# schmidtniko/visual_marker_mapping

Measured on AMD Instinct MI355X. Metric: lm_iterations_per_sec, higher is better.
Workload: dtype f64; 1 GPU; configs[1]: 500 images x 200 tags, visibility 1.00, 100000 tag observations (400000 corner residual blocks), no loss, perturbed initial guess; eliminated_family=cameras, reduced_system_order=1200, elimination_form=dense Z + MFMA rank-k, kept_family_order=natural

## Files before the change

visual_marker_mapping_amd/csrc/kernels_chol.hip:

```cpp
#include <type_traits>
#include <utility>

#include "engine.hpp"

namespace vmm {

#ifdef VMM_STAMPS
__device__ unsigned long long g_stamps[64];
#define STAMP(slot)                                                                  \
    do {                                                                             \
        if (blockIdx.x == 1 && threadIdx.x == 0 && k == 1) {                         \
            g_stamps[slot] = __builtin_amdgcn_s_memtime();                           \
            g_stamps[16 + slot] = __builtin_amdgcn_s_memrealtime();                  \
        }                                                                            \
    } while (0)
#define USTAMP(slot)                                                                 \
    do {                                                                             \
        if (u == 0 && threadIdx.x == 0 && k == 1 && t == u + n_wg)                   \
            g_stamps[(slot)] = __builtin_amdgcn_s_memtime();                         \
    } while (0)
#else
#define USTAMP(slot)
#define STAMP(slot)
#endif
// ... 731 lines not shown
            L[r * kLd + cc] = (cc <= r) ? Ld[(int64_t)kb * 4096 + r * 64 + cc] : 0.0;
        }
        if (tid < 64)
            di[tid] = dinv[K0 + tid];
    }
    __syncthreads();
    if (part == 0) {
        wc = w[m * kNB + c];
        if (kb + 1 < n_blk) {
            wc -= (red[0][c] + red[1][c]) + (red[2][c] + red[3][c]);
            w[m * kNB + c] = wc;
        }
    }
    if (m != kb)
        return;
    double yj = 0.0;
    for (int j0 = 60; j0 >= 0; j0 -= 4) {
        if (part == 0)
            ws[c] = wc;
        __syncthreads();
        if (part == 0) {
            const double* D = L + j0 * kLd + j0;
            const double v3 = ws[j0 + 3] * di[j0 + 3];
            const double v2 = (ws[j0 + 2] - D[3 * kLd + 2] * v3) * di[j0 + 2];
            const double v1 = (ws[j0 + 1] - D[2 * kLd + 1] * v2 - D[3 * kLd + 1] * v3) * di[j0 + 1];
            const double v0 = (ws[j0] - D[kLd] * v1 - D[2 * kLd] * v2 - D[3 * kLd] * v3) * di[j0];
            if (c >= j0 && c < j0 + 4)
                yj = (c == j0) ? v0 : (c == j0 + 1 ? v1 : (c == j0 + 2 ? v2 : v3));
            if (c < j0)
                wc -= L[j0 * kLd + c] * v0 + L[(j0 + 1) * kLd + c] * v1 + L[(j0 + 2) * kLd + c] * v2
                    + L[(j0 + 3) * kLd + c] * v3;
        }
        __syncthreads();
    }
    if (part == 0)
        y[kb * kNB + c] = yj;
}

constexpr unsigned kSpinLimit = 1u << 22;

__device__ __forceinline__ void raise_sync_timeout(LmCtl* ctl, int bit)
{
    atomicOr(&ctl->sync_timeout, bit);
    atomicExch(&ctl->done, 2);
}

int backsolve_chain_workgroups(int n_blk) { return n_blk; }

__device__ __forceinline__ void chain_block_done(unsigned* n_done, int n_blk, unsigned* epoch_word, unsigned epoch,
                                                 bool tree, int m)
{
    if (!tree) {
        if (m == 0)
            *epoch_word = epoch;
        return;
    }
    if (atomicAdd(n_done, 1u) == (unsigned)n_blk - 1u) {
        *n_done = 0u;
        *epoch_word = epoch;
    }
}

#ifdef VMM_STAMPS
__device__ unsigned long long g_chain_stamps[128][4];
#define CH_RT(blk, slot)                                                                  \
    do {                                                                                  \
        if (threadIdx.x == 0)                                                             \
            g_chain_stamps[(blk) & 127][slot] = __builtin_amdgcn_s_memrealtime();         \
    } while (0)
extern "C" int vmm_ba_debug_read_chain_stamps(unsigned long long* out)
{
    return (int)hipMemcpyFromSymbol(out, HIP_SYMBOL(g_chain_stamps), sizeof(unsigned long long) * 128 * 4);
}
#else
#define CH_RT(blk, slot)
#endif

__global__ __launch_bounds__(256) void k_backsolve_chain(LmCtl* ctl, const double* __restrict__ S, int ld,
                                                         int n_pad, int n_blk, double* y,
                                                         const double* __restrict__ dinv, unsigned long long* gran,
                                                         unsigned* epoch_word, const double* __restrict__ Ld,
                                                         const double* __restrict__ Linv)
{
    if (ctl->done || ctl->lin_fail) {
        if (blockIdx.x == gridDim.x - 1 && threadIdx.x == 0)
            *epoch_word = *epoch_word + 1u;
        return;
    }
    const unsigned spin_limit = (ctl->spin_limit_chain && (ctl->spin_wg < 0 || ctl->spin_wg == (int)blockIdx.x))
                                    ? ctl->spin_limit_chain : kSpinLimit;
    __shared__ double L[64 * kLd];
    __shared__ double Li[64 * kLd];
    __shared__ double red[4][64];
    __shared__ double ws[64];
    __shared__ double ys[2][64];
    __shared__ double sB[16][256];
    __shared__ int s_timeout;
    const int m = n_blk - 1 - (int)blockIdx.x;
    const int tid = threadIdx.x;
    const int c = tid & 63, part = tid >> 6;
    const unsigned epoch = *epoch_word + 1u;
    const int K0 = m * kNB;
    if (tid == 0)
        s_timeout = 0;
    CH_RT(m, 0);
    auto receive = [&](const int j, double* ysj) {
        if (part == 0) {
            const unsigned long long* g = gran + 2 * (int64_t)(j * kNB + c);
            unsigned long long x0, x1;
            for (unsigned n = 0;;) {
                x0 = __hip_atomic_load(g, __ATOMIC_RELAXED, __HIP_MEMORY_SCOPE_AGENT);
                x1 = __hip_atomic_load(g + 1, __ATOMIC_RELAXED, __HIP_MEMORY_SCOPE_AGENT);
                const bool ok = (unsigned)(x0 >> 32) == epoch && (unsigned)(x1 >> 32) == epoch;
                if (__all(ok) && spin_limit != 1u)
                    break;
                __builtin_amdgcn_s_sleep(1);
                if (++n >= spin_limit) {
                    s_timeout = 1;
                    break;
                }
            }
            ysj[c] = __longlong_as_double((long long)(((x1 & 0xffffffffull) << 32) | (x0 & 0xffffffffull)));
        }
    };
    auto publish = [&](const double yv) {
        const unsigned long long bits = (unsigned long long)__double_as_longlong(yv);
        const unsigned long long tag = (unsigned long long)epoch << 32;
        unsigned long long* g = gran + 2 * (int64_t)(K0 + c);
        __hip_atomic_store(g, tag | (bits & 0xffffffffull), __ATOMIC_RELAXED, __HIP_MEMORY_SCOPE_AGENT);
        __hip_atomic_store(g + 1, tag | (bits >> 32), __ATOMIC_RELAXED, __HIP_MEMORY_SCOPE_AGENT);
        y[K0 + c] = yv;
    };
    if (m == n_blk - 1) {
        if (part == 0) {
            double lcol[64];
#pragma unroll
            for (int jj = 0; jj < 64; ++jj)
                lcol[jj] = (c <= jj) ? Ld[(int64_t)m * 4096 + jj * 64 + c] : 0.0;
            const double dic = dinv[K0 + c];
            double wv = S[(int64_t)n_pad * ld + K0 + c];
            double yv = 0.0;
#pragma unroll
            for (int jj = 63; jj >= 0; --jj) {
                const long long wb = __double_as_longlong(wv * dic);
                const unsigned w0 = (unsigned)__builtin_amdgcn_readlane((int)wb, jj);
                const unsigned w1 = (unsigned)__builtin_amdgcn_readlane((int)(wb >> 32), jj);
                const double yj = __longlong_as_double((long long)(((unsigned long long)w1 << 32) | w0));
                yv = (c == jj) ? yj : yv;
                wv = (c < jj) ? wv - lcol[jj] * yj : wv;
            }
            publish(yv);
        }
        CH_RT(m, 2);
        if (tid == 0 && m == 0)
            *epoch_word = epoch;
        return;
    }
    double li[16];
    {
        for (int idx = tid; idx < 64 * 64; idx += 256) {
            const int r = idx >> 6, cc = idx & 63;
            L[r * kLd + cc] = S[(int64_t)((m + 1) * kNB + r) * ld + K0 + cc];
            Li[r * kLd + cc] = Linv[(int64_t)m * 4096 + r * 64 + cc];
        }
        __syncthreads();
#pragma unroll
        for (int r = 0; r < 16; ++r)
            li[r] = Li[(part * 16 + r) * kLd + c];
        const int fi = c & 15, fk = c >> 4;
        double4_t accB[4];
#pragma unroll
        for (int t = 0; t < 4; ++t)
            accB[t] = (double4_t){ 0.0, 0.0, 0.0, 0.0 };
#pragma unroll
        for (int ks = 0; ks < 16; ++ks) {
            const double av = L[(part * 16 + fi) * kLd + 4 * ks + fk];
#pragma unroll
            for (int t = 0; t < 4; ++t)
                accB[t] = __builtin_amdgcn_mfma_f64_16x16x4f64(av, Li[(4 * ks + fk) * kLd + 16 * t + fi], accB[t], 0, 0, 0);
        }
#pragma unroll
        for (int t = 0; t < 4; ++t)
#pragma unroll
            for (int r = 0; r < 4; ++r)
                sB[fk + 4 * r][part * 64 + 16 * t + fi] = accB[t][r];
        __syncthreads();
    }
    double acc = 0.0;
    double lt[16], ln[16];
    int j = n_blk - 1;
    if (j > m + 1) {
        const double* Lb = S + (int64_t)(j * kNB + part * 16) * ld + K0 + c;
#pragma unroll
        for (int r = 0; r < 16; ++r)
            lt[r] = Lb[(int64_t)r * ld];
    }
    for (; j > m + 1; --j) {
        if (j - 1 > m + 1) {
            const double* Lb = S + (int64_t)((j - 1) * kNB + part * 16) * ld + K0 + c;
#pragma unroll
            for (int r = 0; r < 16; ++r)
                ln[r] = Lb[(int64_t)r * ld];
        }
        double* ysj = ys[j & 1];
        receive(j, ysj);
        __syncthreads();
#pragma unroll
        for (int r = 0; r < 16; ++r)
            acc += lt[r] * ysj[part * 16 + r];
#pragma unroll
        for (int r = 0; r < 16; ++r)
            lt[r] = ln[r];
    }
    red[part][c] = acc;
    __syncthreads();
    if (part == 0)
        ws[c] = S[(int64_t)n_pad * ld + K0 + c] - ((red[0][c] + red[1][c]) + (red[2][c] + red[3][c]));
    __syncthreads();
    double a2 = 0.0;
#pragma unroll
    for (int r = 0; r < 16; ++r)
        a2 += li[r] * ws[part * 16 + r];
    __syncthreads();
// ... 1515 lines not shown
```

visual_marker_mapping_amd/csrc/kernels_lm.hip:

```cpp
#include <float.h>

#include "engine.hpp"

namespace vmm {

__device__ __forceinline__ void control_reduce(double (&v)[8], double (&m)[2], double* sh)
{
    const int lane = threadIdx.x & 63, wave = threadIdx.x >> 6;
    const int nw = blockDim.x >> 6;
#pragma unroll
    for (int level = 0; level < 3; ++level) {
        const int off = 32 >> level;
        const bool hi = (lane & off) != 0;
#pragma unroll
        for (int j = 0; j < (4 >> level); ++j) {
            const double keep = hi ? v[2 * j + 1] : v[2 * j];
            const double send = hi ? v[2 * j] : v[2 * j + 1];
            v[j] = keep + __shfl_xor(send, off, 64);
        }
    }
#pragma unroll
    for (int off = 4; off >= 1; off >>= 1)
        v[0] += __shfl_xor(v[0], off, 64);
    {
// ... 270 lines not shown
            else
                c.num_unsuccessful++;
            if (c.records < c.trace_capacity)
                trace[c.records] = cur;
            c.records++;
            if (cur.iteration >= c.max_num_iterations) {
                stop = 1;
                c.termination = VMM_BA_NO_CONVERGENCE;
            } else if (cur.step_is_successful && cur.gradient_max_norm <= c.gradient_tolerance) {
                stop = 1;
                c.termination = VMM_BA_CONVERGENCE;
            } else if (c.radius <= c.min_radius) {
                stop = 1;
                c.termination = VMM_BA_CONVERGENCE;
            }
            if (stop) {
                c.done = 1;
            } else {
                vmm_ba_iteration z;
                z.iteration = cur.iteration + 1;
                z.step_is_valid = 0;
                z.step_is_successful = 0;
                z.reserved = 0;
                z.cost = c.x_cost;
                z.cost_change = 0.0;
                z.gradient_max_norm = cur.gradient_max_norm;
                z.step_norm = 0.0;
                z.relative_decrease = 0.0;
                z.trust_region_radius = 0.0;
                z.model_cost_change = 0.0;
                c.cur = z;
                c.iteration = z.iteration;
                c.lin_fail = 0;
                c.num_lm_iterations++;
            }
        }
        s_stop = stop;
        s_accept = accept;
        s_moved = moved;
        s_reuse = c.reuse_diagonal;
        s_radius = c.radius;
        s_lo = c.min_lm_diagonal;
        s_hi = c.max_lm_diagonal;
        if (!stop)
            c.reuse_diagonal = 1;
        else
            c.phase_ticks[1] += span(t_begin, __builtin_amdgcn_s_memrealtime());
        CTL_RT(3);
        *ctl = c;
        CTL_RT(4);
    }
    __syncthreads();
    CTL_RT(5);
    if (s_accept) {
        for (int i = tid; i < 7 * pv.n_cams; i += (int)blockDim.x)
            pv.cam_qt[i] = pv.cam_cand[i];
        for (int i = tid; i < 7 * pv.n_tags; i += (int)blockDim.x)
            pv.tag_qt[i] = pv.tag_cand[i];
    }
    if (staged && s_moved)
        for (size_t i = tid; i < small_count; i += blockDim.x)
            dst[i] = src[i];
    if (s_stop)
        return;
    const double* __restrict__ Hx = s_moved ? Hn : H0 + (which ? alt_off : 0);
    const double lo = s_lo, hi = s_hi;
    for (int q = tid; q < n_tan; q += (int)blockDim.x) {
        double d;
        if (!s_reuse) {
            const int p = q / 6, k = q % 6;
            const double sc = scale[q];
            d = sc * sc * Hx[36 * (int64_t)p + 7 * k];
            d = fmin(fmax(d, lo), hi);
            diag[q] = d;
        } else {
            d = diag[q];
        }
        const double lm = sqrt(d / s_radius);
        D2[q] = lm * lm;
    }
    CTL_RT(6);
}

__device__ __forceinline__ void candidate_for_pose(const PoseViews& pv, const int p, const double (&d)[6],
                                                   double* __restrict__ delta, const double* __restrict__ H,
                                                   const double* __restrict__ g, const int32_t* __restrict__ active,
                                                   double* __restrict__ pose_part)
{
    double bad = 0.0;
#pragma unroll
    for (int k = 0; k < 6; ++k) {
        delta[6 * (int64_t)p + k] = d[k];
        if (!isfinite(d[k]))
            bad = 1.0;
    }
    const double* x = pose_ptr(pv, p, false);
    double out[7];
    block_plus(pv, p, x, d, out);
    double* c = pose_ptr(pv, p, true);
    double sn = 0.0, xn = 0.0;
    for (int k = 0; k < 7; ++k) {
        c[k] = out[k];
        const double df = x[k] - out[k];
        sn += df * df;
        xn += out[k] * out[k];
    }
    const double* Hp = H + 36 * (int64_t)p;
    double gd = 0.0, quad = 0.0;
    for (int a = 0; a < 6; ++a) {
        gd += d[a] * g[6 * (int64_t)p + a];
        double r = 0.0;
        for (int b = 0; b < 6; ++b)
            r += Hp[6 * a + b] * d[b];
        quad += d[a] * r;
    }
    const bool act = active[p] != 0;
    double* o = pose_part + 5 * (int64_t)p;
    o[0] = gd;
    o[1] = quad;
    o[2] = act ? sn : 0.0;
    o[3] = act ? xn : 0.0;
    o[4] = bad;
}

template <bool FUSE, bool SPARSE>
__global__ __launch_bounds__(256) void k_backsub(const LmCtl* ctl, int n_e, int e_off_pose,
                                                 const int32_t* __restrict__ pose_task,
                                                 const double* __restrict__ Z, int ldz, int n_red,
                                                 const double* __restrict__ yf, const double* __restrict__ Le,
                                                 const double* __restrict__ ze, const double* __restrict__ scale,
                                                 double* __restrict__ step_comm, double* __restrict__ part_cross,
                                                 PoseViews pv, int f_off_pose, int n_f, int nb_e,
                                                 double* __restrict__ delta, const double* __restrict__ H0,
                                                 const double* __restrict__ g0, const int64_t alt_off,
                                                 const int32_t* __restrict__ active,
                                                 double* __restrict__ pose_part,
                                                 const int32_t* __restrict__ e_start,
                                                 const int32_t* __restrict__ e_other,
                                                 const int32_t* __restrict__ row_of)
{
    if (!FUSE && blockIdx.x == 0 && threadIdx.x == 0)
        step_comm[7 * (int64_t)n_e] = (ctl->done == 2) ? 1.0 : 0.0;
    if (ctl->done)
        return;
    phase_stamp(ctl, 4);
    const bool lin_fail = ctl->lin_fail != 0;
    const double* __restrict__ H = H0 + small_sel(ctl, alt_off);
    const double* __restrict__ g = g0 + small_sel(ctl, alt_off);
    if (FUSE && (int)blockIdx.x >= nb_e) {
        const int f = ((int)blockIdx.x - nb_e) * blockDim.x + threadIdx.x;
        if (f >= n_f)
            return;
        const int p = f_off_pose + f;
        double d[6];
#pragma unroll
        for (int k = 0; k < 6; ++k)
            d[k] = lin_fail ? 0.0 : -yf[(row_of ? row_of[f] : 6 * f) + k] * scale[6 * (int64_t)p + k];
        candidate_for_pose(pv, p, d, delta, H, g, active, pose_part);
        return;
    }
    const int e = (int)blockIdx.x;
    const int lane = threadIdx.x & 63, wave = threadIdx.x >> 6;
    if (e >= n_e)
        return;
    const bool owned = pose_task[e + 1] > pose_task[e];
    if (!owned || lin_fail) {
        if (wave != 0)
            return;
        if (lane < 6)
            step_comm[6 * (int64_t)e + lane] = 0.0;
        if (lane == 0) {
            part_cross[e] = 0.0;
            if (FUSE) {
                const double d[6] = { 0.0, 0.0, 0.0, 0.0, 0.0, 0.0 };
                candidate_for_pose(pv, e_off_pose + e, d, delta, H, g, active, pose_part);
            }
        }
        return;
    }
    __shared__ double s_acc[4][6];
    double acc[6] = { 0, 0, 0, 0, 0, 0 };
    if (SPARSE) {
        const int es = e_start[e], rs = 6 * (e_start[e + 1] - es);
        const double* zp = Z + 36 * (int64_t)es;
        for (int t = (int)threadIdx.x; t < rs; t += 256) {
            const int k = t / 6, c = t - 6 * k;
            const int fo = e_other[es + k];
            const double yv = yf[(row_of ? row_of[fo] : 6 * fo) + c];
#pragma unroll
            for (int i = 0; i < 6; ++i)
                acc[i] += zp[36 * k + 6 * c + i] * yv;
        }
    } else {
        const double* zr = Z + (int64_t)(6 * e) * ldz;
        for (int c = 2 * (int)threadIdx.x; c < n_red; c += 512) {
            const double2 yv = *reinterpret_cast<const double2*>(yf + c);
#pragma unroll
            for (int i = 0; i < 6; ++i) {
                const double2 zv = *reinterpret_cast<const double2*>(zr + (int64_t)i * ldz + c);
                acc[i] += zv.x * yv.x + zv.y * yv.y;
            }
        }
    }
#pragma unroll
    for (int i = 0; i < 6; ++i) {
        const double a = wave_sum(acc[i]);
        if (lane == 0)
            s_acc[wave][i] = a;
    }
    __syncthreads();
    if (wave != 0)
        return;
    double v[6];
    double cr = 0.0;
#pragma unroll
    for (int i = 0; i < 6; ++i) {
        const double a = (s_acc[0][i] + s_acc[1][i]) + (s_acc[2][i] + s_acc[3][i]);
        v[i] = ze[6 * (int64_t)e + i] - a;
        cr += v[i] * a;
    }
    const double* L = Le + 36 * (int64_t)e;
#pragma unroll
    for (int i = 5; i >= 0; --i) {
        double s = v[i];
#pragma unroll
        for (int k = i + 1; k < 6; ++k)
            s -= L[6 * k + i] * v[k];
        v[i] = s / L[6 * i + i];
    }
    double d[6];
#pragma unroll
    for (int i = 0; i < 6; ++i)
        d[i] = -v[i] * scale[6 * (int64_t)(e_off_pose + e) + i];
    if (lane < 6) {
        double out = 0.0;
#pragma unroll
        for (int i = 0; i < 6; ++i)
            out = (lane == i) ? d[i] : out;
        step_comm[6 * (int64_t)e + lane] = out;
    }
    if (lane == 0) {
        part_cross[e] = cr;
        if (FUSE)
            candidate_for_pose(pv, e_off_pose + e, d, delta, H, g, active, pose_part);
    }
}

__global__ void k_candidate(LmCtl* ctl, PoseViews pv, int n_e, int e_off_pose, int f_off_pose,
                            const double* __restrict__ step_comm, const double* __restrict__ yf,
                            const double* __restrict__ scale, double* __restrict__ delta,
                            const double* __restrict__ H, const double* __restrict__ g,
                            const int32_t* __restrict__ active, double* __restrict__ pose_part,
                            const int32_t* __restrict__ row_of)
{
    const bool remote = step_comm[7 * (int64_t)n_e] > 0.0;
    if (remote && blockIdx.x == 0 && threadIdx.x == 0 && ctl->done != 1) {
        if (ctl->done == 0)
            atomicOr(&ctl->sync_timeout, 4);
        atomicExch(&ctl->done, 2);
    }
    if (ctl->done || remote)
        return;
    const int p = blockIdx.x * blockDim.x + threadIdx.x;
    const int n_pose = pv.n_cams + pv.n_tags;
    if (p >= n_pose)
        return;
    const bool is_e = (p >= e_off_pose) && (p < e_off_pose + n_e);
    double d[6];
    for (int k = 0; k < 6; ++k) {
        if (ctl->lin_fail)
            d[k] = 0.0;
        else if (is_e)
            d[k] = step_comm[6 * (int64_t)(p - e_off_pose) + k];
        else
            d[k] = -yf[(row_of ? row_of[p - f_off_pose] : 6 * (p - f_off_pose)) + k] * scale[6 * (int64_t)p + k];
    }
    candidate_for_pose(pv, p, d, delta, H, g, active, pose_part);
}

__global__ __launch_bounds__(256) void k_begin_loop(LmCtl* ctl, const LmCtl init, const int n_cam7, const int n_tag7,
                                                    const double* __restrict__ stage_cam,
                                                    const double* __restrict__ stage_tag, double* __restrict__ cam_qt,
                                                    double* __restrict__ tag_qt, double* __restrict__ cam_cand,
                                                    double* __restrict__ tag_cand)
{
    const int i = blockIdx.x * blockDim.x + threadIdx.x;
    if (i == 0)
        *ctl = init;
    if (i < n_cam7) {
        double v;
        if (stage_cam) {
            v = stage_cam[i];
            cam_qt[i] = v;
        } else {
            v = cam_qt[i];
        }
        cam_cand[i] = v;
    } else if (i < n_cam7 + n_tag7) {
        const int k = i - n_cam7;
        double v;
        if (stage_tag) {
            v = stage_tag[k];
            tag_qt[k] = v;
        } else {
            v = tag_qt[k];
        }
        tag_cand[k] = v;
    }
}

void launch_begin_loop(Engine& e, const LmCtl& init)
{
    const int n_cam7 = 7 * e.n_cams, n_tag7 = 7 * e.n_tags;
    const double* sc = e.dirty_cam ? e.pose_stage_dev : nullptr;
    const double* st = e.dirty_tag ? e.pose_stage_dev + n_cam7 : nullptr;
    hipLaunchKernelGGL(k_begin_loop, dim3((n_cam7 + n_tag7 + 255) / 256), dim3(256), 0, e.stream, e.ctl, init, n_cam7,
                       n_tag7, sc, st, e.cam_qt, e.tag_qt, e.cam_cand, e.tag_cand);
}

__global__ void k_pose_plus(int64_t n, const double* __restrict__ qt, const double* __restrict__ delta,
                            double* __restrict__ out)
{
    const int64_t i = (int64_t)blockIdx.x * blockDim.x + threadIdx.x;
    if (i >= n)
        return;
    double x[7], d[6], o[7];
    for (int k = 0; k < 7; ++k)
// ... 98 lines not shown
```

visual_marker_mapping_amd/csrc/kernels_schur.hip:

```cpp
#include "engine.hpp"

namespace vmm {


__device__ __forceinline__ bool chol6(double* A)
{
    bool ok = true;
#pragma unroll
    for (int j = 0; j < 6; ++j) {
        double d = A[6 * j + j];
#pragma unroll
        for (int k = 0; k < j; ++k)
            d -= A[6 * j + k] * A[6 * j + k];
        if (!(d > 0.0) || !isfinite(d)) {
            ok = false;
            d = 1.0;
        }
        d = sqrt(d);
        A[6 * j + j] = d;
        const double inv = 1.0 / d;
#pragma unroll
        for (int i = j + 1; i < 6; ++i) {
            double s = A[6 * i + j];
#pragma unroll
            for (int k = 0; k < j; ++k)
                s -= A[6 * i + k] * A[6 * j + k];
            A[6 * i + j] = s * inv;
        }
    }
    return ok;
}

template <typename WT, bool SPARSE>
__global__ __launch_bounds__(256) void k_form_z(LmCtl* ctl, int64_t n_obs, int64_t n_pad,
                                                 const int32_t* __restrict__ own,
                                                 const int32_t* __restrict__ other,
                                                 const WT* __restrict__ W0, const WT* __restrict__ W1,
                                                 const double* __restrict__ H_E0, const double* __restrict__ g_E0,
                                                 const int64_t alt_off,
                                                 const double* __restrict__ D2,
                                                 double* __restrict__ Le, double* __restrict__ ze,
                                                 const double* __restrict__ scale, int e_off_pose,
                                                 int f_off_pose, double* __restrict__ Z, int ldz, int zcol,
                                                 const int32_t* __restrict__ e_start)
{
    if (ctl->done)
        return;
    phase_stamp(ctl, 2);
    const int64_t i = (int64_t)blockIdx.x * blockDim.x + threadIdx.x;
    if (i >= n_obs)
        return;
    const WT* __restrict__ W = ctl->w_which ? W1 : W0;
    const double* __restrict__ H_E = H_E0 + small_sel(ctl, alt_off);
    const double* __restrict__ g_E = g_E0 + small_sel(ctl, alt_off);
    const int e = own[i], f = other[i];
    const double* se = scale + 6 * (int64_t)(e_off_pose + e);
    const double* sf = scale + 6 * (int64_t)(f_off_pose + f);
    double L[36];
    {
        const double* d2 = D2 + 6 * (int64_t)(e_off_pose + e);
#pragma unroll
        for (int a = 0; a < 6; ++a) {
#pragma unroll
            for (int b = 0; b < 6; ++b)
                L[6 * a + b] = se[a] * H_E[36 * (int64_t)e + 6 * a + b] * se[b];
            L[6 * a + a] += d2[a];
        }
    }
    const bool ok = chol6(L);
    const bool first = i == 0 || own[i - 1] != e;
    if (first) {
        if (!ok)
            ctl->lin_fail = 1;
        double v[6];
#pragma unroll
        for (int a = 0; a < 6; ++a)
            v[a] = se[a] * g_E[6 * (int64_t)e + a];
#pragma unroll
        for (int r = 0; r < 6; ++r) {
            double t = v[r];
#pragma unroll
            for (int k = 0; k < r; ++k)
                t -= L[6 * r + k] * v[k];
            v[r] = t / L[6 * r + r];
        }
#pragma unroll
        for (int k = 0; k < 36; ++k)
            Le[36 * (int64_t)e + k] = L[k];
#pragma unroll
        for (int k = 0; k < 6; ++k) {
            ze[6 * (int64_t)e + k] = v[k];
            if (!SPARSE)
                Z[(int64_t)(6 * e + k) * ldz + zcol] = v[k];
        }
    }
    double X[36];
#pragma unroll
    for (int a = 0; a < 6; ++a)
#pragma unroll
        for (int b = 0; b < 6; ++b)
            X[6 * a + b] = se[a] * (double)W[(int64_t)(6 * a + b) * n_pad + i] * sf[b];
#pragma unroll
    for (int r = 0; r < 6; ++r) {
        const double inv = 1.0 / L[6 * r + r];
#pragma unroll
        for (int c = 0; c < 6; ++c) {
            double t = X[6 * r + c];
#pragma unroll
            for (int k = 0; k < r; ++k)
                t -= L[6 * r + k] * X[6 * k + c];
            X[6 * r + c] = t * inv;
        }
    }
    int64_t rs = ldz;
    double* zrow = Z + (int64_t)(6 * e) * ldz + 6 * f;
    if (SPARSE) {
        double* zb = Z + 36 * i;
#pragma unroll
        for (int c = 0; c < 6; ++c)
#pragma unroll
            for (int r = 0; r < 6; ++r)
                zb[6 * c + r] = X[6 * r + c];
        return;
    }
#pragma unroll
    for (int r = 0; r < 6; ++r)
#pragma unroll
        for (int c = 0; c < 6; ++c)
            zrow[(int64_t)r * rs + c] = X[6 * r + c];
}


typedef double double4_t __attribute__((ext_vector_type(4)));

constexpr int kSyrkKT = kKT;
constexpr int kSyrkT = kST;
constexpr int kSyrkRow = 144;
constexpr int kSyrkTile = kSyrkT * kSyrkT;

struct SyrkPlanDev {
    int n_tiles, n_kt, n_wg;
    const int32_t* tile_bi;
    const int32_t* tile_bj;
    const int64_t* wg_u0;
    const int64_t* wg_u1;
    const int32_t* wg_seg0;
    const int32_t* tile_seg0;
    double* partials;
};

__global__ __launch_bounds__(256, 2) void k_syrk_streamk(const LmCtl* ctl, const double* __restrict__ Z, int ldz,
                                                         SyrkPlanDev pl)
{
    if (ctl && ctl->done)
        return;
    __shared__ __attribute__((aligned(16))) double As[2][kSyrkKT * kSyrkRow];
    __shared__ __attribute__((aligned(16))) double Bs[2][kSyrkKT * kSyrkRow];
    const int g = blockIdx.x;
    int64_t u = pl.wg_u0[g];
    const int64_t u_end = pl.wg_u1[g];
    int seg = pl.wg_seg0[g];
    const int tid = threadIdx.x;
    const int lane = tid & 63, wave = tid >> 6;
    const int wi = wave >> 1, wj = wave & 1;
    const int lr = tid >> 5;
    const int lc = (tid & 31) * 4;
    const int fk = lane >> 4, fi = lane & 15;
    while (u < u_end) {
        const int t = (int)(u / pl.n_kt);
        const int kt0 = (int)(u % pl.n_kt);
        const int64_t left = u_end - u;
        const int kt1 = (kt0 + left < pl.n_kt) ? (int)(kt0 + left) : pl.n_kt;
        const int I0 = pl.tile_bi[t] * kSyrkT, J0 = pl.tile_bj[t] * kSyrkT;
        const bool diag = I0 == J0;
        double4_t acc[4][4];
#pragma unroll
        for (int a = 0; a < 4; ++a)
#pragma unroll
            for (int b = 0; b < 4; ++b)
                acc[a][b] = (double4_t){ 0.0, 0.0, 0.0, 0.0 };
        double4_t va[2], vb[2];
        auto gload = [&](int kt) {
#pragma unroll
            for (int h = 0; h < 2; ++h) {
                const double* zr = Z + (int64_t)(kt * kSyrkKT + lr + 8 * h) * ldz;
                va[h] = *reinterpret_cast<const double4_t*>(zr + I0 + lc);
                vb[h] = *reinterpret_cast<const double4_t*>(zr + J0 + lc);
            }
        };
        auto lstore = [&](int buf) {
#pragma unroll
            for (int h = 0; h < 2; ++h) {
                *reinterpret_cast<double4_t*>(&As[buf][(lr + 8 * h) * kSyrkRow + lc]) = va[h];
                *reinterpret_cast<double4_t*>(&Bs[buf][(lr + 8 * h) * kSyrkRow + lc]) = vb[h];
            }
        };
        gload(kt0);
        __syncthreads();
        lstore(0);
        __syncthreads();
        const bool live = !(diag && wi == 0 && wj == 1);
        for (int kt = kt0; kt < kt1; ++kt) {
            const int buf = (kt - kt0) & 1;
            if (kt + 1 < kt1)
                gload(kt + 1);
            const double* Ap = As[buf];
            const double* Bp = Bs[buf];
            if (live) {
#pragma unroll
                for (int ks = 0; ks < kSyrkKT / 4; ++ks) {
                    const int row = (ks * 4 + fk) * kSyrkRow;
                    double a[4], b[4];
// ... 80 lines not shown
        }
    };
    struct Frag {
        double a[T::NA], b[T::NB];
    };
    auto read_ops = [&](const int buf, const int ks, Frag& f) {
        const double* Ap = Ag + buf * 2 * kGStage;
        const double* Bp = DIAG ? Ap : Ap + kGStage;
        const int row = (ks * 4 + fk) * kSyrkRow;
#pragma unroll
        for (int i = 0; i < T::NA; ++i)
            f.a[i] = Ap[row + 16 * T::arow(i) + fi];
#pragma unroll
        for (int j = 0; j < T::NB; ++j)
            f.b[j] = Bp[row + 16 * T::bcol(j) + fi];
    };
    auto mfma_step = [&](const Frag& f) {
#pragma unroll
        for (int n = 0; n < T::NT; ++n)
            acc[n] = __builtin_amdgcn_mfma_f64_16x16x4f64(f.a[T::ai(n)], f.b[T::bi(n)], acc[n], 0, 0, 0);
    };
    if (my_n > 0) {
        gload(0);
        lstore(0);
    }
    if (g == 1)
        __syncthreads();
    for (int i = 0; i < n0; ++i) {
        __syncthreads();
        const bool have = i < my_n, more = i + 1 < my_n;
        const int buf = i & 1;
        Frag f0, f1, f2;
        if (more)
            gload(i + 1);
        if (have) {
            read_ops(buf, 0, f0);
            read_ops(buf, 1, f1);
            mfma_step(f0);
            read_ops(buf, 2, f2);
            mfma_step(f1);
        }
        __syncthreads();
        if (have) {
            mfma_step(f2);
            read_ops(buf, 3, f0);
            mfma_step(f0);
        }
        if (more)
            lstore(buf ^ 1);
    }
    if (g == 0)
        __syncthreads();
    __syncthreads();
    constexpr int H = T::NT / 2;
    double* const X = smem + (size_t)W * 16 * 256;
#pragma unroll
    for (int n = 0; n < T::NT; ++n)
        if ((n < H) == (g == 1)) {
#pragma unroll
            for (int r = 0; r < 4; ++r)
                X[(n * 4 + r) * 64 + lane] = acc[n][r];
        }
    __syncthreads();
#pragma unroll
    for (int n = 0; n < T::NT; ++n)
        if ((n < H) == (g == 0)) {
            const int tr = T::arow(T::ai(n)), tc = T::bcol(T::bi(n));
            double v[4];
#pragma unroll
            for (int r = 0; r < 4; ++r) {
                v[r] = acc[n][r] + X[(n * 4 + r) * 64 + lane];
                Cb[(16 * tr + fk + 4 * r) * kSyrkT + 16 * tc + fi] = v[r];
            }
            if (DIAG && tr > tc && (tr >> 2) == (tc >> 2)) {
#pragma unroll
                for (int r = 0; r < 4; ++r)
                    Cb[(16 * tc + fi) * kSyrkT + 16 * tr + fk + 4 * r] = v[r];
            }
        }
}

__global__ __launch_bounds__(512, 1) void k_syrk_wide(const LmCtl* ctl, const double* __restrict__ Z, int ldz, SyrkPlanDev pl)
{
    if (ctl && ctl->done)
        return;
    __shared__ __attribute__((aligned(16))) double smem[4 * kWideStage];
    static_assert(4 * kWideStage >= 4 * 16 * 256, "the accumulator exchange must fit into the stage buffers");
    const int gidx = blockIdx.x;
    const int64_t u = pl.wg_u0[gidx], u_end = pl.wg_u1[gidx];
    if (u >= u_end)
        return;
    const int t = (int)(u / pl.n_kt);
    const int kt0 = (int)(u % pl.n_kt), kt1 = kt0 + (int)(u_end - u);
    const int I0 = pl.tile_bi[t] * kSyrkT, J0 = pl.tile_bj[t] * kSyrkT;
    double* Cb = pl.partials + (size_t)pl.wg_seg0[gidx] * kSyrkTile;
    const int w = __builtin_amdgcn_readfirstlane((int)(threadIdx.x >> 6) & 3);
    if (I0 == J0) {
        switch (w) {
        case 0: syrk_wide_item<true, 0>(Z, ldz, I0, J0, kt0, kt1, smem, Cb); break;
        case 1: syrk_wide_item<true, 1>(Z, ldz, I0, J0, kt0, kt1, smem, Cb); break;
        case 2: syrk_wide_item<true, 2>(Z, ldz, I0, J0, kt0, kt1, smem, Cb); break;
        default: syrk_wide_item<true, 3>(Z, ldz, I0, J0, kt0, kt1, smem, Cb); break;
        }
    } else {
        switch (w) {
        case 0: syrk_wide_item<false, 0>(Z, ldz, I0, J0, kt0, kt1, smem, Cb); break;
        case 1: syrk_wide_item<false, 1>(Z, ldz, I0, J0, kt0, kt1, smem, Cb); break;
        case 2: syrk_wide_item<false, 2>(Z, ldz, I0, J0, kt0, kt1, smem, Cb); break;
        default: syrk_wide_item<false, 3>(Z, ldz, I0, J0, kt0, kt1, smem, Cb); break;
        }
    }
}

struct DiagArgs {
    const double* H_F;
    const double* g_F;
    const double* scale_F;
    const double* D2_F;
    int n_red, n_pad;
    int64_t alt_off;
};

template <bool ADD_DIAG>
__global__ __launch_bounds__(256) void k_reduce_partials(const LmCtl* ctl, SyrkPlanDev pl, int ld, int n_rows,
                                                         double* __restrict__ S, DiagArgs da,
                                                         double* __restrict__ packed = nullptr)
{
    if (ctl && ctl->done)
        return;
    const int t = blockIdx.x >> 4;
    const int sub = blockIdx.x & 15;
    const int qi = sub >> 3, qj = (sub >> 2) & 1, rs = sub & 3;
    const int I0 = pl.tile_bi[t] * kSyrkT + 64 * qi, J0 = pl.tile_bj[t] * kSyrkT + 64 * qj;
    if (J0 > I0 || I0 + 16 * rs >= n_rows)
        return;
    const int s0 = pl.tile_seg0[t], s1 = pl.tile_seg0[t + 1];
    const int tr = 16 * rs + (threadIdx.x >> 5), tc = (threadIdx.x & 31) * 2;
    if (ADD_DIAG && ctl) {
        da.H_F += small_sel(ctl, da.alt_off);
        da.g_F += small_sel(ctl, da.alt_off);
    }
    double2 acc[2] = { make_double2(0.0, 0.0), make_double2(0.0, 0.0) };
    const double* p0 = pl.partials + (size_t)(64 * qi + tr) * kSyrkT + 64 * qj + tc;
#pragma unroll 4
    for (int q = s0; q < s1; ++q) {
        const double* pq = p0 + (size_t)q * kSyrkTile;
#pragma unroll
        for (int i = 0; i < 2; ++i) {
            const double2 v = *reinterpret_cast<const double2*>(pq + 8 * i * kSyrkT);
            acc[i].x += v.x;
            acc[i].y += v.y;
        }
    }
#pragma unroll
    for (int i = 0; i < 2; ++i) {
        const int row = I0 + tr + 8 * i;
        if (row >= n_rows)
            continue;
        double out[2] = { -acc[i].x, -acc[i].y };
#pragma unroll
        for (int h = 0; h < 2; ++h) {
            const int col = J0 + tc + h;
            double v = out[h];
            if (ADD_DIAG) {
                if (row == da.n_pad) {
                    if (col < da.n_red)
                        v += da.scale_F[col] * da.g_F[col];
                } else if (row < da.n_red && col <= row && (row / 6) == (col / 6)) {
                    const int f = row / 6, a = row % 6, b = col % 6;
                    v += da.scale_F[row] * da.H_F[36 * (int64_t)f + 6 * a + b] * da.scale_F[col];
                    if (a == b)
                        v += da.D2_F[row];
                } else if (row >= da.n_red && row < da.n_pad && col == row) {
                    v = 1.0;
                }
            }
            out[h] = v;
        }
// ... 454 lines not shown
```

Before: 2467 LM iterations/s.

## Hoist operand loads before control checks and stage form_z stores through LDS

Several kernels now issue their global loads (pose operands, Cholesky factors, scales, plan entries, chain back-solve inputs) before reading the control word. This lets the load latency overlap the control-flag read. In k_form_z, the per-pose 6x6 Cholesky is computed once by the head thread and shared through an LDS table with the other threads of the same pose, instead of every observation refactoring it. The Z block writes are restaged through LDS so the stores go out as coalesced double2 accesses. In exchange, these kernels do extra loads even when the solver is done, add barriers, and use more LDS and registers.

```diff
diff --git a/visual_marker_mapping_amd/csrc/kernels_chol.hip b/visual_marker_mapping_amd/csrc/kernels_chol.hip
--- a/visual_marker_mapping_amd/csrc/kernels_chol.hip
+++ b/visual_marker_mapping_amd/csrc/kernels_chol.hip
@@ -837,6 +837,16 @@
                                                          unsigned* epoch_word, const double* __restrict__ Ld,
                                                          const double* __restrict__ Linv)
 {
+    double lcol[64];
+    double dic = 0.0, wv = 0.0;
+    if (blockIdx.x == 0 && threadIdx.x < 64) {
+        const int mt = n_blk - 1, ct = (int)threadIdx.x;
+#pragma unroll
+        for (int jj = 0; jj < 64; ++jj)
+            lcol[jj] = (ct <= jj) ? Ld[(int64_t)mt * 4096 + jj * 64 + ct] : 0.0;
+        dic = dinv[mt * kNB + ct];
+        wv = S[(int64_t)n_pad * ld + mt * kNB + ct];
+    }
     if (ctl->done || ctl->lin_fail) {
         if (blockIdx.x == gridDim.x - 1 && threadIdx.x == 0)
             *epoch_word = *epoch_word + 1u;
@@ -888,12 +898,6 @@
     };
     if (m == n_blk - 1) {
         if (part == 0) {
-            double lcol[64];
-#pragma unroll
-            for (int jj = 0; jj < 64; ++jj)
-                lcol[jj] = (c <= jj) ? Ld[(int64_t)m * 4096 + jj * 64 + c] : 0.0;
-            const double dic = dinv[K0 + c];
-            double wv = S[(int64_t)n_pad * ld + K0 + c];
             double yv = 0.0;
 #pragma unroll
             for (int jj = 63; jj >= 0; --jj) {
diff --git a/visual_marker_mapping_amd/csrc/kernels_lm.hip b/visual_marker_mapping_amd/csrc/kernels_lm.hip
--- a/visual_marker_mapping_amd/csrc/kernels_lm.hip
+++ b/visual_marker_mapping_amd/csrc/kernels_lm.hip
@@ -376,45 +376,76 @@
     CTL_RT(6);
 }
 
+struct PoseOperands {
+    double x[7], H[36], g[6];
+    bool act;
+};
+
+__device__ __forceinline__ void load_pose_operands(const PoseViews& pv, const int p, const double* __restrict__ H,
+                                                   const double* __restrict__ g, const int32_t* __restrict__ active,
+                                                   PoseOperands& o)
+{
+    const double* x = pose_ptr(pv, p, false);
+#pragma unroll
+    for (int k = 0; k < 7; ++k)
+        o.x[k] = x[k];
+#pragma unroll
+    for (int k = 0; k < 36; ++k)
+        o.H[k] = H[36 * (int64_t)p + k];
+#pragma unroll
+    for (int k = 0; k < 6; ++k)
+        o.g[k] = g[6 * (int64_t)p + k];
+    o.act = active[p] != 0;
+}
+
+__device__ __forceinline__ void candidate_from_operands(const PoseViews& pv, const int p, const double (&d)[6],
+                                                        double* __restrict__ delta, const PoseOperands& po,
+                                                        double* __restrict__ pose_part)
+{
+    double bad = 0.0;
+#pragma unroll
+    for (int k = 0; k < 6; ++k) {
+        delta[6 * (int64_t)p + k] = d[k];
+        if (!isfinite(d[k]))
+            bad = 1.0;
+    }
+    double out[7];
+    block_plus(pv, p, po.x, d, out);
+    double* c = pose_ptr(pv, p, true);
+    double sn = 0.0, xn = 0.0;
+#pragma unroll
+    for (int k = 0; k < 7; ++k) {
+        c[k] = out[k];
+        const double df = po.x[k] - out[k];
+        sn += df * df;
+        xn += out[k] * out[k];
+    }
+    double gd = 0.0, quad = 0.0;
+#pragma unroll
+    for (int a = 0; a < 6; ++a) {
+        gd += d[a] * po.g[a];
+        double r = 0.0;
+#pragma unroll
+        for (int b = 0; b < 6; ++b)
+            r += po.H[6 * a + b] * d[b];
+        quad += d[a] * r;
+    }
+    double* o = pose_part + 5 * (int64_t)p;
+    o[0] = gd;
+    o[1] = quad;
+    o[2] = po.act ? sn : 0.0;
+    o[3] = po.act ? xn : 0.0;
+    o[4] = bad;
+}
+
 __device__ __forceinline__ void candidate_for_pose(const PoseViews& pv, const int p, const double (&d)[6],
                                                    double* __restrict__ delta, const double* __restrict__ H,
                                                    const double* __restrict__ g, const int32_t* __restrict__ active,
                                                    double* __restrict__ pose_part)
 {
-    double bad = 0.0;
-#pragma unroll
-    for (int k = 0; k < 6; ++k) {
-        delta[6 * (int64_t)p + k] = d[k];
-        if (!isfinite(d[k]))
-            bad = 1.0;
-    }
-    const double* x = pose_ptr(pv, p, false);
-    double out[7];
-    block_plus(pv, p, x, d, out);
-    double* c = pose_ptr(pv, p, true);
-    double sn = 0.0, xn = 0.0;
-    for (int k = 0; k < 7; ++k) {
-        c[k] = out[k];
-        const double df = x[k] - out[k];
-        sn += df * df;
-        xn += out[k] * out[k];
-    }
-    const double* Hp = H + 36 * (int64_t)p;
-    double gd = 0.0, quad = 0.0;
-    for (int a = 0; a < 6; ++a) {
-        gd += d[a] * g[6 * (int64_t)p + a];
-        double r = 0.0;
-        for (int b = 0; b < 6; ++b)
-            r += Hp[6 * a + b] * d[b];
-        quad += d[a] * r;
-    }
-    const bool act = active[p] != 0;
-    double* o = pose_part + 5 * (int64_t)p;
-    o[0] = gd;
-    o[1] = quad;
-    o[2] = act ? sn : 0.0;
-    o[3] = act ? xn : 0.0;
-    o[4] = bad;
+    PoseOperands po;
+    load_pose_operands(pv, p, H, g, active, po);
+    candidate_from_operands(pv, p, d, delta, po, pose_part);
 }
 
 template <bool FUSE, bool SPARSE>
@@ -435,12 +466,18 @@
 {
     if (!FUSE && blockIdx.x == 0 && threadIdx.x == 0)
         step_comm[7 * (int64_t)n_e] = (ctl->done == 2) ? 1.0 : 0.0;
-    if (ctl->done)
+    int task0 = 0, task1 = 0;
+    if ((int)blockIdx.x < n_e) {
+        task0 = pose_task[blockIdx.x];
+        task1 = pose_task[blockIdx.x + 1];
+    }
+    const int done = ctl->done, lin_fail_w = ctl->lin_fail, which = ctl->w_which;
+    if (done)
         return;
     phase_stamp(ctl, 4);
-    const bool lin_fail = ctl->lin_fail != 0;
-    const double* __restrict__ H = H0 + small_sel(ctl, alt_off);
-    const double* __restrict__ g = g0 + small_sel(ctl, alt_off);
+    const bool lin_fail = lin_fail_w != 0;
+    const double* __restrict__ H = H0 + (which ? alt_off : 0);
+    const double* __restrict__ g = g0 + (which ? alt_off : 0);
     if (FUSE && (int)blockIdx.x >= nb_e) {
         const int f = ((int)blockIdx.x - nb_e) * blockDim.x + threadIdx.x;
         if (f >= n_f)
@@ -457,7 +494,7 @@
     const int lane = threadIdx.x & 63, wave = threadIdx.x >> 6;
     if (e >= n_e)
         return;
-    const bool owned = pose_task[e + 1] > pose_task[e];
+    const bool owned = task1 > task0;
     if (!owned || lin_fail) {
         if (wave != 0)
             return;
@@ -473,6 +510,22 @@
         return;
     }
     __shared__ double s_acc[4][6];
+    double zv0[6], Lt[36], sc0[6];
+    PoseOperands po;
+    if (wave == 0) {
+#pragma unroll
+        for (int i = 0; i < 6; ++i) {
+            zv0[i] = ze[6 * (int64_t)e + i];
+            sc0[i] = scale[6 * (int64_t)(e_off_pose + e) + i];
+        }
+#pragma unroll
+        for (int k = 0; k < 6; ++k)
+#pragma unroll
+            for (int i = 0; i <= k; ++i)
+                Lt[6 * k + i] = Le[36 * (int64_t)e + 6 * k + i];
+        if (FUSE)
+            load_pose_operands(pv, e_off_pose + e, H, g, active, po);
+    }
     double acc[6] = { 0, 0, 0, 0, 0, 0 };
     if (SPARSE) {
         const int es = e_start[e], rs = 6 * (e_start[e + 1] - es);
@@ -510,10 +563,10 @@
 #pragma unroll
     for (int i = 0; i < 6; ++i) {
         const double a = (s_acc[0][i] + s_acc[1][i]) + (s_acc[2][i] + s_acc[3][i]);
-        v[i] = ze[6 * (int64_t)e + i] - a;
+        v[i] = zv0[i] - a;
         cr += v[i] * a;
     }
-    const double* L = Le + 36 * (int64_t)e;
+    const double* L = Lt;
 #pragma unroll
     for (int i = 5; i >= 0; --i) {
         double s = v[i];
@@ -525,7 +578,7 @@
     double d[6];
 #pragma unroll
     for (int i = 0; i < 6; ++i)
-        d[i] = -v[i] * scale[6 * (int64_t)(e_off_pose + e) + i];
+        d[i] = -v[i] * sc0[i];
     if (lane < 6) {
         double out = 0.0;
 #pragma unroll
@@ -536,7 +589,7 @@
     if (lane == 0) {
         part_cross[e] = cr;
         if (FUSE)
-            candidate_for_pose(pv, e_off_pose + e, d, delta, H, g, active, pose_part);
+            candidate_from_operands(pv, e_off_pose + e, d, delta, po, pose_part);
     }
 }
 
diff --git a/visual_marker_mapping_amd/csrc/kernels_schur.hip b/visual_marker_mapping_amd/csrc/kernels_schur.hip
--- a/visual_marker_mapping_amd/csrc/kernels_schur.hip
+++ b/visual_marker_mapping_amd/csrc/kernels_schur.hip
@@ -30,6 +30,10 @@
     }
     return ok;
 }
+
+constexpr int kFormZPoses = 64;
+constexpr int kFormZSlot = 42;
+constexpr int kFormZStageRow = 384;
 
 template <typename WT, bool SPARSE>
 __global__ __launch_bounds__(256) void k_form_z(LmCtl* ctl, int64_t n_obs, int64_t n_pad,
@@ -44,20 +48,41 @@
                                                  int f_off_pose, double* __restrict__ Z, int ldz, int zcol,
                                                  const int32_t* __restrict__ e_start)
 {
-    if (ctl->done)
+    constexpr int kTable = kFormZPoses * kFormZSlot;
+    constexpr int kStage = SPARSE ? 0 : 4 * 6 * kFormZStageRow;
+    __shared__ __attribute__((aligned(16))) double lds[kStage > kTable ? kStage : kTable];
+    const int tid = (int)threadIdx.x;
+    const int64_t i0 = (int64_t)blockIdx.x * blockDim.x;
+    const int64_t i = i0 + tid;
+    const bool valid = i < n_obs;
+    int e = valid ? own[i] : 0, f = valid ? other[i] : 0;
+    int e_prev = (valid && i > 0) ? own[i - 1] : -1, e_wg = own[i0];
+    const int done = ctl->done, which = ctl->w_which;
+    asm volatile("" : "+v"(e), "+v"(f), "+v"(e_prev), "+v"(e_wg));
+    if (done)
         return;
     phase_stamp(ctl, 2);
-    const int64_t i = (int64_t)blockIdx.x * blockDim.x + threadIdx.x;
-    if (i >= n_obs)
-        return;
-    const WT* __restrict__ W = ctl->w_which ? W1 : W0;
-    const double* __restrict__ H_E = H_E0 + small_sel(ctl, alt_off);
-    const double* __restrict__ g_E = g_E0 + small_sel(ctl, alt_off);
-    const int e = own[i], f = other[i];
+    const WT* __restrict__ W = which ? W1 : W0;
+    const double* __restrict__ H_E = H_E0 + (which ? alt_off : 0);
+    const double* __restrict__ g_E = g_E0 + (which ? alt_off : 0);
+    const int slot = e - e_wg;
+    const bool use_table = __syncthreads_and(!valid || (slot >= 0 && slot < kFormZPoses)) != 0;
+    const bool head = valid && (tid == 0 || e_prev != e);
+    const bool first = valid && (i == 0 || e_prev != e);
     const double* se = scale + 6 * (int64_t)(e_off_pose + e);
     const double* sf = scale + 6 * (int64_t)(f_off_pose + f);
-    double L[36];
-    {
+    double X[36];
+    auto load_block = [&]() {
+#pragma unroll
+        for (int a = 0; a < 6; ++a)
+#pragma unroll
+            for (int b = 0; b < 6; ++b)
+                X[6 * a + b] = se[a] * (double)W[(int64_t)(6 * a + b) * n_pad + i] * sf[b];
+    };
+    if (!SPARSE && valid)
+        load_block();
+    double L[36], inv[6];
+    if (valid && (head || !use_table)) {
         const double* d2 = D2 + 6 * (int64_t)(e_off_pose + e);
 #pragma unroll
         for (int a = 0; a < 6; ++a) {
@@ -66,55 +91,77 @@
                 L[6 * a + b] = se[a] * H_E[36 * (int64_t)e + 6 * a + b] * se[b];
             L[6 * a + a] += d2[a];
         }
-    }
-    const bool ok = chol6(L);
-    const bool first = i == 0 || own[i - 1] != e;
-    if (first) {
-        if (!ok)
-            ctl->lin_fail = 1;
-        double v[6];
-#pragma unroll
-        for (int a = 0; a < 6; ++a)
-            v[a] = se[a] * g_E[6 * (int64_t)e + a];
+        const bool ok = chol6(L);
+        if (first) {
+            if (!ok)
+                ctl->lin_fail = 1;
+            double v[6];
+#pragma unroll
+            for (int a = 0; a < 6; ++a)
+                v[a] = se[a] * g_E[6 * (int64_t)e + a];
+#pragma unroll
+            for (int r = 0; r < 6; ++r) {
+                double t = v[r];
+#pragma unroll
+                for (int k = 0; k < r; ++k)
+                    t -= L[6 * r + k] * v[k];
+                v[r] = t / L[6 * r + r];
+            }
+#pragma unroll
+            for (int k = 0; k < 36; ++k)
+                Le[36 * (int64_t)e + k] = L[k];
+#pragma unroll
+            for (int k = 0; k < 6; ++k) {
+                ze[6 * (int64_t)e + k] = v[k];
+                if (!SPARSE)
+                    Z[(int64_t)(6 * e + k) * ldz + zcol] = v[k];
+            }
+        }
+#pragma unroll
+        for (int r = 0; r < 6; ++r)
+            inv[r] = 1.0 / L[6 * r + r];
+        if (use_table) {
+            double* t = lds + slot * kFormZSlot;
+#pragma unroll
+            for (int r = 0; r < 6; ++r) {
+#pragma unroll
+                for (int k = 0; k < r; ++k)
+                    t[6 * r + k] = L[6 * r + k];
+                t[36 + r] = inv[r];
+            }
+        }
+    }
+    if (use_table) {
+        __syncthreads();
+        if (valid && !head) {
+            const double* t = lds + slot * kFormZSlot;
+#pragma unroll
+            for (int r = 0; r < 6; ++r) {
+#pragma unroll
+                for (int k = 0; k < r; ++k)
+                    L[6 * r + k] = t[6 * r + k];
+                inv[r] = t[36 + r];
+            }
+        }
+    }
+    if (valid) {
+        if (SPARSE)
+            load_block();
 #pragma unroll
         for (int r = 0; r < 6; ++r) {
-            double t = v[r];
-#pragma unroll
-            for (int k = 0; k < r; ++k)
-                t -= L[6 * r + k] * v[k];
-            v[r] = t / L[6 * r + r];
-        }
-#pragma unroll
-        for (int k = 0; k < 36; ++k)
-            Le[36 * (int64_t)e + k] = L[k];
-#pragma unroll
-        for (int k = 0; k < 6; ++k) {
-            ze[6 * (int64_t)e + k] = v[k];
-            if (!SPARSE)
-                Z[(int64_t)(6 * e + k) * ldz + zcol] = v[k];
-        }
-    }
-    double X[36];
-#pragma unroll
-    for (int a = 0; a < 6; ++a)
-#pragma unroll
-        for (int b = 0; b < 6; ++b)
-            X[6 * a + b] = se[a] * (double)W[(int64_t)(6 * a + b) * n_pad + i] * sf[b];
-#pragma unroll
-    for (int r = 0; r < 6; ++r) {
-        const double inv = 1.0 / L[6 * r + r];
-#pragma unroll
-        for (int c = 0; c < 6; ++c) {
-            double t = X[6 * r + c];
-#pragma unroll
-            for (int k = 0; k < r; ++k)
-                t -= L[6 * r + k] * X[6 * k + c];
-            X[6 * r + c] = t * inv;
-        }
-    }
-    int64_t rs = ldz;
-    double* zrow = Z + (int64_t)(6 * e) * ldz + 6 * f;
+#pragma unroll
+            for (int c = 0; c < 6; ++c) {
+                double t = X[6 * r + c];
+#pragma unroll
+                for (int k = 0; k < r; ++k)
+                    t -= L[6 * r + k] * X[6 * k + c];
+                X[6 * r + c] = t * inv[r];
+            }
+        }
+    }
     if (SPARSE) {
+        if (!valid)
+            return;
         double* zb = Z + 36 * i;
 #pragma unroll
         for (int c = 0; c < 6; ++c)
@@ -123,11 +170,31 @@
                 zb[6 * c + r] = X[6 * r + c];
         return;
     }
-#pragma unroll
-    for (int r = 0; r < 6; ++r)
-#pragma unroll
-        for (int c = 0; c < 6; ++c)
-            zrow[(int64_t)r * rs + c] = X[6 * r + c];
+    const int lane = tid & 63;
+    double* st = lds + (tid >> 6) * (6 * kFormZStageRow);
+    __syncthreads();
+    if (valid) {
+#pragma unroll
+        for (int r = 0; r < 6; ++r)
+#pragma unroll
+            for (int c = 0; c < 6; c += 2)
+                *reinterpret_cast<double2*>(st + r * kFormZStageRow + 6 * lane + c) = make_double2(X[6 * r + c], X[6 * r + c + 1]);
+    }
+    __syncthreads();
+#pragma unroll
+    for (int k = 0; k < 3; ++k) {
+        const int p = lane + 64 * k;
+        const int src = p / 3, cc = 2 * (p - 3 * src);
+        const int es = __shfl(e, src), fs = __shfl(f, src);
+        const bool vs = __shfl((int)valid, src) != 0;
+        if (vs) {
+            double* zp = Z + (int64_t)(6 * es) * ldz + 6 * fs + cc;
+#pragma unroll
+            for (int r = 0; r < 6; ++r)
+                *reinterpret_cast<double2*>(zp + (int64_t)r * ldz) =
+                    *reinterpret_cast<const double2*>(st + r * kFormZStageRow + 2 * p);
+        }
+    }
 }
 
 
@@ -374,18 +441,19 @@
 
 __global__ __launch_bounds__(512, 1) void k_syrk_wide(const LmCtl* ctl, const double* __restrict__ Z, int ldz, SyrkPlanDev pl)
 {
-    if (ctl && ctl->done)
-        return;
     __shared__ __attribute__((aligned(16))) double smem[4 * kWideStage];
     static_assert(4 * kWideStage >= 4 * 16 * 256, "the accumulator exchange must fit into the stage buffers");
     const int gidx = blockIdx.x;
     const int64_t u = pl.wg_u0[gidx], u_end = pl.wg_u1[gidx];
+    const int seg0 = pl.wg_seg0[gidx];
+    if (ctl && ctl->done)
+        return;
     if (u >= u_end)
         return;
     const int t = (int)(u / pl.n_kt);
     const int kt0 = (int)(u % pl.n_kt), kt1 = kt0 + (int)(u_end - u);
     const int I0 = pl.tile_bi[t] * kSyrkT, J0 = pl.tile_bj[t] * kSyrkT;
-    double* Cb = pl.partials + (size_t)pl.wg_seg0[gidx] * kSyrkTile;
+    double* Cb = pl.partials + (size_t)seg0 * kSyrkTile;
     const int w = __builtin_amdgcn_readfirstlane((int)(threadIdx.x >> 6) & 3);
     if (I0 == J0) {
         switch (w) {
```

Result: no change. 2480 LM iterations/s, median of 3 (+0.5%).
